# Eden-Kramer-Lab/spectral_connectivity

Measured on AMD Instinct MI355X. Metric: channel-pair*freq-bins/s for CSM+coherence(+wPLI), higher is better.
Workload: dtype f32

## Files before the change

### spectral_connectivity_amd/_build.py

```python
import hashlib
import os
import shutil
import subprocess
import sys
from concurrent.futures import ThreadPoolExecutor

HERE = os.path.dirname(os.path.abspath(__file__))
CSRC = os.path.join(HERE, "csrc")
LIB = os.path.join(HERE, "libsc_hip.so")
OBJ_DIR = os.path.join(os.path.dirname(HERE), "build", "obj")
SOURCES = ["sc_api.hip", "sc_taper.hip", "sc_mtfft.hip", "sc_mtfft_long.hip", "sc_mtfft_mixed.hip", "sc_mtfft_f64.hip", "sc_csm.hip", "sc_nonlinear.hip", "sc_fused.hip", "sc_fused2.hip", "sc_measure.hip",
           "sc_wilson.hip", "sc_wilson_fft.hip", "sc_wilson_pair.hip", "sc_mvar.hip", "sc_conditional.hip", "sc_blockwise.hip", "sc_global.hip", "sc_canonical.hip", "sc_partial.hip", "sc_jackknife.hip", "sc_f64.hip",
           "sc_timing.hip", "sc_memory.hip", "sc_comm.hip"]
HEADERS = ["sc_common.h", "sc_stage.h", "sc_fused_common.h", "sc_fused_plan.h", "sc_jacobi.h", "sc_wilson_fft.h", "sc_wilson_loop.h", "sc_complex.h", "sc_mtfft_bfly.h", os.path.join("..", "..", "include", "sc_hip.h")]
FLAGS = ["-O3", "-std=c++17", "--offload-arch=gfx950", "-fPIC", "-Wno-unused-result", "-fno-slp-vectorize"]


def _hipcc():
    for cand in (os.environ.get("HIPCC"), shutil.which("hipcc"), "/opt/rocm/bin/hipcc"):
        if cand and os.path.exists(cand):
            return cand
    raise RuntimeError("hipcc not found: cannot build libsc_hip.so (set HIPCC=/path/to/hipcc)")


def sources():
    return [os.path.join(CSRC, s) for s in SOURCES if os.path.exists(os.path.join(CSRC, s))]


def is_stale():
# ... 55 lines not shown
```

### spectral_connectivity_amd/csrc/sc_api.hip

```cpp
#include <stdarg.h>
#include <stdlib.h>
#include <string.h>
#include <rocfft/rocfft.h>
#include "sc_common.h"

static thread_local char g_err[512] = "";

void sc_set_error(const char* fmt, ...) {
    va_list ap;
    va_start(ap, fmt);
    vsnprintf(g_err, sizeof(g_err), fmt, ap);
    va_end(ap);
}

static const char* const g_switch_names[SC_SW_COUNT] = {
    "SC_FUSED_DEBUG", "SC_FUSED2_TERMS", "SC_FUSED_SPLIT", "SC_FUSED_NO_SMALL", "SC_MTFFT_DEBUG", "SC_MTFFT_WIDE", "SC_MTFFT_F64",
    "SC_F64_SPLIT", "SC_F64_OC", "SC_F64_NO_FORK", "SC_F64_NO_BLOCK", "SC_WILSON_FFT", "SC_GLOBAL_EIG", "SC_GLOBAL_NT256",
    "SC_GRANGER_KERNEL", "SC_FUSED_FOLD_OBS", "SC_MTFFT_LONG", "SC_CANON_EIG", "SC_MTFFT_MIXED", "SC_MTFFT_MIXED_GEO", "SC_MTFFT_SLICE", "SC_MVAR_INVERSE"};
static char g_switch_val[SC_SW_COUNT][32];
static bool g_switch_set[SC_SW_COUNT];
extern "C" int sc_debug_reload_env(void) {
    for (int i = 0; i < SC_SW_COUNT; ++i) {
        const char* v = getenv(g_switch_names[i]);
        g_switch_set[i] = v != nullptr;
        if (v) { strncpy(g_switch_val[i], v, sizeof(g_switch_val[i]) - 1); g_switch_val[i][sizeof(g_switch_val[i]) - 1] = 0; }
    }
    return SC_OK;
}
static const int g_switches_loaded = sc_debug_reload_env();
const char* sc_switch(int id) { return (id >= 0 && id < SC_SW_COUNT && g_switch_set[id]) ? g_switch_val[id] : nullptr; }

#include <mutex>
#include <vector>
// ... 254 lines not shown
```

### spectral_connectivity_amd/csrc/sc_common.h

```cpp
#pragma once
#include <hip/hip_runtime.h>
#include <stdint.h>
#include <stdio.h>
#include "../../include/sc_hip.h"
#include "sc_complex.h"

void sc_set_error(const char* fmt, ...);
struct ScRec;
struct ScCsmView;

enum ScSwitch {
    SC_SW_FUSED_DEBUG, SC_SW_FUSED2_TERMS, SC_SW_FUSED_SPLIT, SC_SW_FUSED_NO_SMALL, SC_SW_MTFFT_DEBUG, SC_SW_MTFFT_WIDE,
    SC_SW_MTFFT_F64, SC_SW_F64_SPLIT, SC_SW_F64_OC, SC_SW_F64_NO_FORK, SC_SW_F64_NO_BLOCK, SC_SW_WILSON_FFT, SC_SW_GLOBAL_EIG,
    SC_SW_GLOBAL_NT256, SC_SW_GRANGER_KERNEL, SC_SW_FUSED_FOLD_OBS, SC_SW_MTFFT_LONG, SC_SW_CANON_EIG, SC_SW_MTFFT_MIXED, SC_SW_MTFFT_MIXED_GEO, SC_SW_MTFFT_SLICE, SC_SW_MVAR_INVERSE, SC_SW_COUNT
};
const char* sc_switch(int id);

int sc_internal_rows_to_bins(const void* d_Z, void* d_X, int64_t rows, int64_t F, int64_t batch, int64_t b_off,
                             int64_t nyquist_row, hipStream_t st);

bool sc_internal_mtfft_long_applies(int64_t N, int64_t C, int64_t groups);
int64_t sc_internal_mtfft_long_coverage(int64_t N, int64_t C);
int sc_internal_mtfft_long(const float* d_x, int64_t T, int64_t R, int64_t C, int64_t L, int64_t step, int64_t W, int64_t N,
                           const float* d_tapers, int64_t K, int detrend_type, const void* d_twiddles, void* d_X, void* d_P,
                           const float* d_scale, hipStream_t st);

bool sc_internal_mtfft_mix_has(int64_t N);
bool sc_internal_mtfft_mix_applies(int64_t N, int64_t C, int64_t groups);
int64_t sc_internal_mtfft_mix_coverage(int64_t N, int64_t C, bool planes);
// ... 237 lines not shown
```

### spectral_connectivity_amd/csrc/sc_fused.hip

```cpp
#include <stdlib.h>
#include "sc_stage.h"
#include "sc_fused_common.h"

#ifdef FU_TRACE
__device__ unsigned long long fu_trace_buf[12 * 4];
#define FU_T0() unsigned long long fu_t = __builtin_readcyclecounter()
#define FU_TICK(slot)                                                                  \
    do {                                                                               \
        const unsigned long long fu_n = __builtin_readcyclecounter();                  \
        if (blockIdx.x == 0 && (threadIdx.x & 63) == 0) fu_trace_buf[(threadIdx.x >> 6) * 4 + (slot)] += fu_n - fu_t; \
        fu_t = fu_n;                                                                   \
    } while (0)
extern "C" int sc_debug_fused_trace(unsigned long long* out, int reset) {
    if (out) (void)hipMemcpyFromSymbol(out, HIP_SYMBOL(fu_trace_buf), sizeof(unsigned long long) * 48);
    if (reset) { unsigned long long z[48] = {0}; (void)hipMemcpyToSymbol(HIP_SYMBOL(fu_trace_buf), z, sizeof z); }
    return 0;
}
#else
#define FU_T0() do {} while (0)
#define FU_TICK(slot) do {} while (0)
#endif

#define FU_PLANE 36
#define FU_CSTRIDE 220
// ... 379 lines not shown
    constexpr int wps = 8 / NSETS;
    const int set = vw / wps, rsub = vw % wps;
    if constexpr (NSETS == 1) {
        fused_valu_body<NB32, COL_LO, ROW_HI, 0, OP>(p, st, planes, raw, tid, vw, rsub, wps, rec, o_lo);
    } else {
        if (set == 0) fused_valu_body<NB32, COL_LO, ROW_HI, 0, OP>(p, st, planes, raw, tid, vw, rsub, wps, rec, o_lo);
        else fused_valu_body<NB32, COL_LO, ROW_HI, 1, OP>(p, st, planes, raw, tid, vw, rsub, wps, rec, o_lo);
    }
}

template <int NB32, int COL_LO, int ROW_HI, int OP>
__global__ void __launch_bounds__(FU_THREADS) fused_csm_absim_kernel(FusedArgs p) {
    extern __shared__ __align__(16) unsigned char smem[];
    const int tid = threadIdx.x;
    const int wave = __builtin_amdgcn_readfirstlane(tid >> 6);
    const int bin = blockIdx.x / p.n_split, part = blockIdx.x - bin * p.n_split;
    const int g = bin / p.F, f = bin - g * p.F;
    ScStage st = p.st;
    st.base = p.st.base + (int64_t)f * st.ax.sF + sc_group_offset(st.ax, g);
    const int nc = (p.st.n_obs + FU_OC - 1) / FU_OC;
    const int o_lo = (int)((int64_t)part * nc / p.n_split) * FU_OC;
    const int o_hi = (int)((int64_t)(part + 1) * nc / p.n_split) * FU_OC;
    st.n_obs = o_hi < p.st.n_obs ? o_hi : p.st.n_obs;
    float* rec = (part == 0 ? p.accum : p.ws + (int64_t)(part - 1) * p.n_bins * p.floats_per_bin) +
                 (int64_t)bin * p.floats_per_bin;
    unsigned short* planes = reinterpret_cast<unsigned short*>(smem);
    constexpr size_t plane_bytes = (size_t)2 * NB32 * 32 * FU_CSTRIDE * 2;
    constexpr size_t red_bytes = (size_t)4 * FU_MAXB * 16 * 64 * sizeof(float);
    float* raw = reinterpret_cast<float*>(smem + (plane_bytes > red_bytes ? plane_bytes : red_bytes));
    if (wave < 4) {
        if (p.debug_skip & 32) __builtin_amdgcn_s_setprio(2);
        fused_mfma_role<NB32>(p, st, planes, raw, tid, wave, rec, o_lo);
    } else {
        if (p.debug_skip & 16) __builtin_amdgcn_s_setprio(2);
        fused_valu_role<NB32, COL_LO, ROW_HI, OP>(p, st, planes, raw, tid, wave - 4, rec, o_lo);
    }
}

__global__ void __launch_bounds__(256) fused_fold_kernel(FusedArgs p) {
    const int64_t plane = (int64_t)p.n_tiles * SC_TILE_ELEMS;
// ... 35 lines not shown
        SC_CHECK_HIP(hipGetLastError());
        return SC_OK;
    }
};

#define SM_THREADS 448
#define SM_CHUNK_BYTES (24 * 1024)

template <bool ABS, bool SQ, bool SGN>
struct SmallSlots { static constexpr int NQ = 2 + (ABS ? 1 : 0) + (SQ ? 1 : 0) + (SGN ? 1 : 0); };

template <bool ABS, bool SQ, bool SGN, bool NORM>
__global__ void __launch_bounds__(SM_THREADS) small_csm_absim_kernel(FusedArgs p) {
    extern __shared__ __align__(16) unsigned char smem[];
    const int tid = threadIdx.x;
    const int bin = blockIdx.x / p.n_split, part = blockIdx.x - bin * p.n_split;
    const int g = bin / p.F, f = bin - g * p.F;
    ScStage st = p.st;
    st.base = p.st.base + (int64_t)f * st.ax.sF + sc_group_offset(st.ax, g);
    const int nc32 = (p.st.n_obs + FU_OC - 1) / FU_OC;
    const int o_lo = (int)((int64_t)part * nc32 / p.n_split) * FU_OC;
    int o_hi = (int)((int64_t)(part + 1) * nc32 / p.n_split) * FU_OC;
    if (o_hi > p.st.n_obs) o_hi = p.st.n_obs;
    float* rec = (part == 0 ? p.accum : p.ws + (int64_t)(part - 1) * p.n_bins * p.floats_per_bin) +
                 (int64_t)bin * p.floats_per_bin;

    const int C = st.C, B = C >> 1, nbk = B * (B + 1) / 2;
    const int S = SM_THREADS / nbk;
    const int s = tid / nbk, b = tid - s * nbk;
    const bool active = s < S;
    int bi = 0, bj = 0;
    { int rem = b, len = B; while (rem >= len) { rem -= len; ++bi; --len; } bj = bi + rem; }
    const int RS = 2 * C;
    const int half = C >> 1;
    int OC = SM_CHUNK_BYTES / (RS * 4);
    OC -= OC % S;
    if (OC > 16 * S) OC = 16 * S;
    const int per_thread = OC / S;
    float* buf0 = reinterpret_cast<float*>(smem);
    float* buf1 = buf0 + (size_t)OC * RS;
// ... 138 lines not shown

static bool fused_ok(const void* d_X, const ScAxes& ax) {
    if (ax.C < 1 || ax.C > 256 || (ax.C & 1)) return false;
    if ((ax.sW | ax.sR | ax.sK | ax.sF) & 1) return false;
    return d_X == nullptr || (((uintptr_t)d_X) % 16 == 0);
}

static bool small_ok(const ScAxes& ax, bool nonlinear_plane) { return ax.C <= (nonlinear_plane ? 48 : 42); }
static bool small_ok_sq(const ScAxes& ax) { return ax.C <= 58; }
static bool small_ok_sign(const ScAxes& ax) { return ax.C <= 44; }

extern "C" int sc_fused_supported(int64_t n_signals) {
    return (n_signals >= 2 && n_signals <= 256 && (n_signals % 2) == 0) ? 1 : 0;
}

int sc_internal_fused_pick_split(int n_bins, int n_obs) {
    const char* e = sc_switch(SC_SW_FUSED_SPLIT);
    const int nc = (n_obs + FU_OC - 1) / FU_OC;
    static int cu_of_device[64] = {0};
    int dev = 0, n_cu = 256;
    if (hipGetDevice(&dev) == hipSuccess && dev >= 0 && dev < 64) {
        if (cu_of_device[dev] == 0) {
            int v = 0;
            cu_of_device[dev] = (hipDeviceGetAttribute(&v, hipDeviceAttributeMultiprocessorCount, dev) == hipSuccess && v > 0) ? v : 256;
        }
        n_cu = cu_of_device[dev];
    }
    int best = 1;
    double best_cost = 1e30;
    for (int S = 1; S <= 24; ++S) {
        if (S > 1 && nc / S < 16) break;
        const double rounds = (double)(((int64_t)n_bins * S + n_cu - 1) / n_cu);
        const double cost = rounds * ((double)nc / S + 3.0) * (1.0 + 0.02 * (S - 1));
        if (cost < best_cost - 1e-9) { best_cost = cost; best = S; }
    }
    if (e && atoi(e) >= 1 && atoi(e) <= 24 && (atoi(e) == 1 || nc / atoi(e) >= 1)) best = atoi(e);
    return best;
}
int sc_internal_fused_set_parts(FusedArgs* a, int n_obs, void* d_workspace, int64_t workspace_bytes) {
    int S = d_workspace ? sc_internal_fused_pick_split(a->n_bins, n_obs) : 1;
    while (S > 1 && (int64_t)(S - 1) * fu_part_bytes(*a) > workspace_bytes) --S;
    SC_REQUIRE(S == 1 || ((uintptr_t)d_workspace % 16) == 0, "workspace must be 16-byte aligned");
    a->n_split = S;
    a->ws = (float*)d_workspace;
    return SC_OK;
}

void sc_internal_fu_assign_rows(FusedArgs* a) {
    const int NB = a->NB, col_lo = a->map.col_lo;
    const int R = a->map.row_hi < NB ? a->map.row_hi : NB;
    auto c0 = [&](int r) { return r > col_lo ? r : col_lo; };
    unsigned packed[4];
    a->seg_n = 0u;
    for (int w = 0; w < 4; ++w) {
        int sg[6] = {0, 0, 0, 0, 0, 0};
        if (R >= 5) {
            const int rA = w, rB = R - 1 - w;
            if (rA <= rB) { sg[0] = rA; sg[1] = c0(rA); sg[2] = NB - c0(rA); }
// ... 52 lines not shown
    } else if (mode == FU_MODE_SIGN) {
        a->csm_plane = a->abs_plane = a->sq_plane = -1;
    } else {
        a->sign_plane = -1;
        if (a->abs_plane < 0) a->sq_plane = -1;
    }
    fu_headline_fold(a);
    return SC_OK;
}

extern "C" int64_t sc_fused_workspace_bytes(const sc_spectra_desc* desc, uint32_t planes) {
    FusedArgs a;
    ScAxes ax;
    const int mode = (planes & SC_PLANE_CSM) ? FU_MODE_CSM : (planes & SC_PLANE_UNIT) ? FU_MODE_UNIT : FU_MODE_SIGN;
    if (fused_setup(nullptr, desc, planes, mode, &a, &ax) != SC_OK) return 0;
    return (int64_t)(sc_internal_fused_pick_split(a.n_bins, ax.n_obs) - 1) * fu_part_bytes(a);
}

static int fused_run(const void* d_X, const sc_spectra_desc* desc, uint32_t planes, int mode, float* d_accum,
                     void* d_workspace, int64_t workspace_bytes, void* d_scratch, int64_t scratch_bytes, void* stream) {
    ScTimed timed_("fused_stage_b", stream);
    SC_REQUIRE(d_X && desc && d_accum, "NULL argument");
    FusedArgs a;
    ScAxes ax;
    const bool unit = mode == FU_MODE_UNIT;
    const int rc = fused_setup(d_X, desc, planes, mode, &a, &ax);
    if (rc != SC_OK) return rc;
    a.accum = d_accum;
    a.st.base = (const float2*)d_X;
    a.st.ax = ax;
    a.st.obs_stride = sc_stage_linear_stride(ax);
// ... 58 lines not shown
```

### spectral_connectivity_amd/csrc/sc_fused2.hip

```cpp
#include <stdlib.h>
#include "sc_fused_common.h"

typedef _Float16 h16x4 __attribute__((ext_vector_type(4)));
typedef _Float16 h16x8 __attribute__((ext_vector_type(8)));
typedef _Float16 h16x2 __attribute__((ext_vector_type(2)));
typedef __attribute__((address_space(3))) unsigned char lds_u8;
typedef short s16x4 __attribute__((ext_vector_type(4)));
typedef __attribute__((address_space(3))) s16x4 lds_s16x4;

#define F2_GROUP 1056
#define F2_PLANE (8 * F2_GROUP + 64)
#define F2_NPL 6
#define F2_HPL 4
#define F2_BUF (F2_NPL * F2_PLANE)
#define F2_NBUF 3
#define F2_SCALE_OFF (F2_NBUF * F2_BUF)
#define F2_LDS (F2_SCALE_OFF + 512)
#define F2_ROW_TILE 256

extern "C" int64_t sc_planes_scales_work_bytes(int64_t n_rows, int64_t width);
extern "C" int64_t sc_planes_row_bytes(int64_t n_signals) { return (int64_t)F2_ROW_TILE * ((n_signals + 31) / 32); }

__device__ __forceinline__ unsigned f2_pack(float lo, float hi) {
    const h16x2 v = {(_Float16)lo, (_Float16)hi};
// ... 617 lines not shown
        const double cyc = (double)(h[s * 4 + 2] - h[s * 4]), ticks = (double)(h[s * 4 + 3] - h[s * 4 + 1]);
        if (ticks > 0 && cyc > 0) { sum += cyc / (ticks / 100.0e6) * 1e-9; ++n; }
    }
    if (ghz) *ghz = n ? sum / n : 0.0;
    return SC_OK;
}

template <int NB32, int COL_LO, int ROW_HI, int OP>
__global__ void __launch_bounds__(FU_THREADS) fused2_kernel(Fused2Args a) {
    extern __shared__ __align__(16) unsigned char smem[];
    const FusedArgs& p = a.f;
    const int tid = threadIdx.x;
    const int wave = __builtin_amdgcn_readfirstlane(tid >> 6);
    const int clock_slot = blockIdx.x == 0 ? 0 : (blockIdx.x == gridDim.x / 2 ? 1 : (blockIdx.x == gridDim.x - 1 ? 2 : -1));
    if (clock_slot >= 0 && tid == 0) f2_clock_stamp(clock_slot, 0);
    const int bin = blockIdx.x / p.n_split, part = blockIdx.x - bin * p.n_split;
    const int g = bin / p.F, f = bin - g * p.F;
    const int nc = (p.st.n_obs + FU_OC - 1) / FU_OC;
    const int o_lo = (int)((int64_t)part * nc / p.n_split) * FU_OC;
    int o_hi = (int)((int64_t)(part + 1) * nc / p.n_split) * FU_OC;
    if (o_hi > p.st.n_obs) o_hi = p.st.n_obs;
    const int n_part = o_hi - o_lo;
    float* rec = (part == 0 ? p.accum : p.ws + (int64_t)(part - 1) * p.n_bins * p.floats_per_bin) + (int64_t)bin * p.floats_per_bin;
    const unsigned char* part_base = a.P + ((int64_t)f * p.st.ax.sF + sc_group_offset(p.st.ax, g) + (int64_t)o_lo * a.obs_rows) * a.row_bytes;
    lds_u8* lds = (lds_u8*)smem;
    constexpr int NHALF = NB32 <= 2 ? 2 : 1, CH = FU_OC * NHALF;
    const F2Loader L = f2_loader<NHALF>(a, wave, part_base);
    for (int i = tid * 16; i < F2_SCALE_OFF; i += FU_THREADS * 16)
        *reinterpret_cast<u32x4*>(smem + i) = (u32x4){0u, 0u, 0u, 0u};
    if (tid < 128) {
        const int gch = fu_byte(p.map.off32, tid >> 5) * 32 + (tid & 31);
        reinterpret_cast<float*>(smem + F2_SCALE_OFF)[tid] = ((tid >> 5) < p.NB32 && (tid & 31) < fu_byte(p.map.n32, tid >> 5) && gch < p.st.C)
                                                                 ? a.inv_scale[gch] : 1.f;
    }
    __syncthreads();
    f2_issue<NHALF>(a, L, lds, 0, n_part);
    const bool second = n_part > CH && !(p.debug_skip & 8);
    if (second) f2_issue<NHALF>(a, L, lds + F2_BUF, CH, n_part - CH);
// ... 144 lines not shown
```

### spectral_connectivity_amd/csrc/sc_fused_common.h

```cpp
#pragma once
#include "sc_stage.h"
#include "sc_fused_plan.h"

typedef float f32x4 __attribute__((ext_vector_type(4)));
typedef short bf16x8 __attribute__((ext_vector_type(8)));
typedef unsigned int u32x4 __attribute__((ext_vector_type(4)));
typedef float f32x2 __attribute__((ext_vector_type(2)));
typedef float f32x16 __attribute__((ext_vector_type(16)));

#define FU_OC 32
#define FU_THREADS 768
#define FU_MAXB 5
#define FU_FLUSH 16

struct FuMap {
    unsigned off32, n32, t32;
    int NBr;
    int col_lo, row_hi;
};
__host__ __device__ inline int fu_byte(unsigned packed, int b) { return (int)((packed >> (8 * b)) & 0xffu); }
__host__ __device__ inline int fu_gt(const FuMap& m, int b) { return fu_byte(m.t32, b >> 1) + (b & 1); }
__host__ __device__ inline bool fu_tile_ok(const FuMap& m, int b) { return (b & 1) * 16 < fu_byte(m.n32, b >> 1); }

struct FusedArgs {
    ScStage st;
    FuMap map;
    float* accum;
    int64_t floats_per_bin;
    int n_bins, F, NB, n_tiles, NB32, n_blocks32, n_sets;
    int shape_col_lo, shape_row_hi;
    int csm_plane, abs_plane;
    int sq_plane, sign_plane;
    int fold[6], n_fold;
    int nl_op;
    unsigned seg0, seg1, seg2, seg3, seg_n;
    int n_split;
    float* ws;
    int debug_skip;
};

__device__ __forceinline__ unsigned cvt_pk_bf16(float lo, float hi) {
    unsigned r;
    asm("v_cvt_pk_bf16_f32 %0, %1, %2" : "=v"(r) : "v"(lo), "v"(hi));
    return r;
}
__device__ __forceinline__ float bf16lo_to_f32(unsigned p) { return __uint_as_float(p << 16); }
__device__ __forceinline__ float bf16hi_to_f32(unsigned p) { return __uint_as_float(p & 0xffff0000u); }

__device__ __forceinline__ void split4(const float x[4], uint2& h, uint2& m, uint2& l) {
    h.x = cvt_pk_bf16(x[0], x[1]); h.y = cvt_pk_bf16(x[2], x[3]);
    const float r0 = x[0] - bf16lo_to_f32(h.x), r1 = x[1] - bf16hi_to_f32(h.x);
    const float r2 = x[2] - bf16lo_to_f32(h.y), r3 = x[3] - bf16hi_to_f32(h.y);
    m.x = cvt_pk_bf16(r0, r1); m.y = cvt_pk_bf16(r2, r3);
    const float s0 = r0 - bf16lo_to_f32(m.x), s1 = r1 - bf16hi_to_f32(m.x);
    const float s2 = r2 - bf16lo_to_f32(m.y), s3 = r3 - bf16hi_to_f32(m.y);
    l.x = cvt_pk_bf16(s0, s1); l.y = cvt_pk_bf16(s2, s3);
}

__device__ __forceinline__ int fu_lane() {
    int l;
    asm volatile("v_mbcnt_lo_u32_b32 %0, -1, 0\n\tv_mbcnt_hi_u32_b32 %0, -1, %0" : "=v"(l));
    return l;
}
enum { FU_OP_ABS = 0, FU_OP_SQ = 1, FU_OP_SIGN = 2, FU_OP_UNIT = 3 };

#define FU_BARRIER() asm volatile("s_waitcnt lgkmcnt(0)\n\ts_barrier" ::: "memory")
#define F2_BARRIER() FU_BARRIER()
static_assert(2 * 4 + 1 <= FU_FLUSH, "one fold slot per tile of a wave");

__host__ __device__ constexpr int fu_nblocks(int nb32, int col_lo, int row_hi) {
    int n = 0;
    for (int bi = 0; bi < nb32 && bi < row_hi; ++bi)
        for (int bj = bi > col_lo ? bi : col_lo; bj < nb32; ++bj) ++n;
    return n;
}
__host__ __device__ constexpr int fu_nsets(int nb32, int col_lo, int row_hi) {
    return fu_nblocks(nb32, col_lo, row_hi) > 4 ? 2 : 1;
// ... 62 lines not shown
#pragma unroll
        for (int e = 0; e < 16; ++e) acc[e] = fu_accumulate<OP>(acc[e], d[e]);
    } else {
        acc[0] = fu_accumulate<OP>(acc[0], d[0]);
        __builtin_amdgcn_sched_barrier(0);
#pragma unroll
        for (int e = 1; e < 16; ++e) {
            int a = __float_as_int(acc[e]), t;
            asm("v_med3_i32 %1, %2, -1, 1\n\tv_add_u32 %0, %0, %1" : "+v"(a), "=&v"(t) : "v"(d[e]));
            acc[e] = __int_as_float(a);
        }
    }
}


int sc_internal_fused_pick_split(int n_bins, int n_obs);
int sc_internal_fused_set_parts(FusedArgs* a, int n_obs, void* d_workspace, int64_t workspace_bytes);
void sc_internal_fu_assign_rows(FusedArgs* a);
int sc_internal_fused_combine(const FusedArgs& a, hipStream_t stream);

inline int64_t fu_part_bytes(const FusedArgs& a) { return (int64_t)a.n_bins * a.floats_per_bin * (int64_t)sizeof(float); }

inline void fu_record_geometry(FusedArgs* a, const ScAxes& ax, uint32_t planes) {
    auto offset = [&](uint32_t plane) { return (planes & plane) ? sc_plane_offset(planes, plane) : -1; };
    a->NB = sc_n_blocks(ax.C);
    a->n_tiles = sc_n_tiles(a->NB);
    a->NB32 = (ax.C + 31) / 32;
    a->map.NBr = a->NB;
    a->n_bins = ax.n_groups * ax.F;
    a->F = ax.F;
    a->floats_per_bin = (int64_t)sc_plane_count(planes) * a->n_tiles * SC_TILE_ELEMS;
    a->csm_plane = offset(SC_PLANE_CSM);
    a->abs_plane = offset(SC_PLANE_ABS_IM);
    a->sq_plane = offset(SC_PLANE_IM_SQ);
    a->sign_plane = offset(SC_PLANE_SIGN_IM);
    a->nl_op = FU_OP_ABS;
    a->n_split = 1;
    a->ws = nullptr;
}
inline void fu_headline_fold(FusedArgs* a) {
    a->n_fold = 0;
    if (a->csm_plane >= 0) { a->fold[a->n_fold++] = a->csm_plane; a->fold[a->n_fold++] = a->csm_plane + 1; }
    if (a->abs_plane >= 0) a->fold[a->n_fold++] = a->abs_plane;
}
inline FusedArgs fu_plane_pass(const FusedArgs& a, int plane, int op) {
    FusedArgs b = a;
    b.csm_plane = -1;
    b.abs_plane = plane;
    b.nl_op = op;
    b.fold[0] = plane;
    b.n_fold = 1;
    return b;
// ... 53 lines not shown
```

### spectral_connectivity_amd/csrc/sc_measure.hip

```cpp
#include <math.h>
#include "sc_common.h"

#define SC_EPS64 2.220446049250313e-16

template <typename AccT>
struct RecT {
    const AccT* p;
    __device__ RecT operator+(int64_t n) const { return RecT{p + n}; }
    __device__ double operator[](int64_t i) const { return (double)p[i]; }
};

template <typename AccT>
struct RecPartsT {
    const AccT* p;
    const AccT* q;
    int n_parts;
    int64_t stride;
    __device__ RecPartsT operator+(int64_t n) const { return RecPartsT{p + n, q + n, n_parts, stride}; }
    __device__ double operator[](int64_t i) const {
        AccT s = p[i];
        for (int k = 1; k < n_parts; ++k) s += q[i + (k - 1) * stride];
        return (double)s;
    }
};

struct MeasureArgs {
    ScRec accum;
    int n_parts;
    const void* rest;
    int64_t part_stride;
    void* out;
    int64_t n_bins, floats_per_bin, total;
    int C, NB, n_tiles;
    int p_csm, p_abs, p_sq, p_sign, p_unit;
    double n_obs, rn_obs;
    int measure;
    int n_multi;
    int multi[SC_MEASURE_MULTI_MAX];
    void* multi_out[SC_MEASURE_MULTI_MAX];
};

template <typename Rec>
__device__ inline double tile_read(Rec bin_rec, int plane, int n_tiles, int NB, int i, int j,
                                  bool* mirrored) {
    int ti = i >> 4, tj = j >> 4, ii = i & 15, jj = j & 15;
    bool m = (ti > tj) || (ti == tj && ii > jj);
    if (m) { int t = ti; ti = tj; tj = t; t = ii; ii = jj; jj = t; }
    *mirrored = m;
    return bin_rec[((int64_t)plane * n_tiles + sc_tile_index(ti, tj, NB)) * SC_TILE_ELEMS + ii * 16 + jj];
}

template <typename AccT, bool PARTS> struct RecSel { using type = RecT<AccT>; };
template <typename AccT> struct RecSel<AccT, true> { using type = RecPartsT<AccT>; };
template <typename AccT, bool PARTS>
// ... 126 lines not shown
    if (i < a.C && j < a.C) {
        if (COMPLEX_OUT) outc[obase + (int64_t)i * a.C + j] = OutT2{(OutT)direct.x, (OutT)direct.y};
        else outf[obase + (int64_t)i * a.C + j] = (OutT)direct.x;
    }
    if (!dtile) {
        mir[jj * 16 + ii] = measure_value(a.measure, a.n_obs, a.rn_obs, measure_mirror(v), false);
        __syncthreads();
        const int r = tj * 16 + ii, c = ti * 16 + jj;
        if (r < a.C && c < a.C) {
            if (COMPLEX_OUT) outc[obase + (int64_t)r * a.C + c] = OutT2{(OutT)mir[tid].x, (OutT)mir[tid].y};
            else outf[obase + (int64_t)r * a.C + c] = (OutT)mir[tid].x;
        }
    }
}

#ifndef MEASURE_MULTI_TPW
#define MEASURE_MULTI_TPW 1
#endif
template <typename OutT, typename AccT, bool PARTS = false>
__global__ void __launch_bounds__(256) measure_tile_multi_kernel(MeasureArgs a) {
    __shared__ MeasureIn raw[256];
    __shared__ double mir[256];
    const int tid = threadIdx.x, ii = tid >> 4, jj = tid & 15;
    const int64_t bin = blockIdx.x;
    using Rec = typename RecSel<AccT, PARTS>::type;
    const Rec rec = make_rec<AccT, PARTS>(a) + bin * a.floats_per_bin;
    const int64_t plane = (int64_t)a.n_tiles * SC_TILE_ELEMS;
    const int64_t obase = bin * (int64_t)a.C * a.C;
    int ti = 0, len = a.NB, t = blockIdx.y * MEASURE_MULTI_TPW;
    while (t >= len) { t -= len; ++ti; --len; }
    for (int u = 0; u < MEASURE_MULTI_TPW; ++u) {
        const int tile_id = blockIdx.y * MEASURE_MULTI_TPW + u;
        if (tile_id >= a.n_tiles) break;
        const int tj = ti + t;
        const Rec tile = rec + ((int64_t)tile_id * SC_TILE_ELEMS + ii * 16 + jj);
        MeasureIn v = {0, 0, 0, 0, 0, 0, 0, 0, 0};
        if (a.p_csm >= 0) {
            v.s_re = (double)tile[a.p_csm * plane];
            v.s_im = (double)tile[(a.p_csm + 1) * plane];
            v.p_i = (double)rec[a.p_csm * plane + (int64_t)sc_tile_index(ti, ti, a.NB) * SC_TILE_ELEMS + ii * 17];
            v.p_j = (double)rec[a.p_csm * plane + (int64_t)sc_tile_index(tj, tj, a.NB) * SC_TILE_ELEMS + jj * 17];
        }
        if (a.p_abs >= 0) v.sa = (double)tile[a.p_abs * plane];
        if (a.p_sq >= 0) v.sq = (double)tile[a.p_sq * plane];
        if (a.p_sign >= 0) v.sg = (double)tile[a.p_sign * plane];
        if (a.p_unit >= 0) {
            v.u_re = (double)tile[a.p_unit * plane];
            v.u_im = (double)tile[(a.p_unit + 1) * plane];
        }
        const bool dtile = ti == tj;
        if (dtile) {
            raw[tid] = v;
            __syncthreads();
            if (ii > jj) v = measure_mirror(raw[jj * 16 + ii]);
            __syncthreads();
        }
        const int i = ti * 16 + ii, j = tj * 16 + jj;
        for (int m = 0; m < a.n_multi; ++m) {
            OutT* outf = (OutT*)a.multi_out[m];
            const int w = a.multi[m];
#ifdef MEASURE_AB_NOMATH
            const double direct = v.s_re + v.sa + w;
#else
            const double direct = measure_value(w, a.n_obs, a.rn_obs, v, i == j).x;
#endif
            if (i < a.C && j < a.C) outf[obase + (int64_t)i * a.C + j] = (OutT)direct;
            if (!dtile) {
                const double sgn = (w == SC_M_COHERENCE_PHASE || w == SC_M_PLI || w == SC_M_WPLI) ? -1.0 : 1.0;
                mir[jj * 16 + ii] = sgn * direct;
                __syncthreads();
                const int r = tj * 16 + ii, c = ti * 16 + jj;
                if (r < a.C && c < a.C) outf[obase + (int64_t)r * a.C + c] = (OutT)mir[tid];
                __syncthreads();
            }
        }
        if (++t >= len) { t = 0; ++ti; --len; }
    }
}

static uint32_t measure_needs(int measure) {
    switch (measure) {
    case SC_M_POWER: case SC_M_CSM: case SC_M_COHERENCY: case SC_M_COHERENCE_MAGNITUDE:
    case SC_M_COHERENCE_PHASE: case SC_M_IMAGINARY_COHERENCE: return SC_PLANE_CSM;
    case SC_M_PLV: case SC_M_PLV_COMPLEX: case SC_M_PPC: return SC_PLANE_UNIT;
    case SC_M_PLI: case SC_M_DEBIASED_PLI2: return SC_PLANE_SIGN_IM;
    case SC_M_WPLI: return SC_PLANE_CSM | SC_PLANE_ABS_IM;
    case SC_M_DEBIASED_WPLI2: return SC_PLANE_CSM | SC_PLANE_ABS_IM | SC_PLANE_IM_SQ;
    }
    return 0;
}

// ... 34 lines not shown
    a.n_multi = n_measures;
    if ((planes & need) != need) {
        sc_set_error("measures need accumulator planes 0x%x, record has 0x%x", need, planes);
        return SC_EINVAL;
    }
    a.p_csm = (need & SC_PLANE_CSM) ? sc_plane_offset(planes, SC_PLANE_CSM) : -1;
    a.p_abs = (need & SC_PLANE_ABS_IM) ? sc_plane_offset(planes, SC_PLANE_ABS_IM) : -1;
    a.p_sq = (need & SC_PLANE_IM_SQ) ? sc_plane_offset(planes, SC_PLANE_IM_SQ) : -1;
    a.p_sign = (need & SC_PLANE_SIGN_IM) ? sc_plane_offset(planes, SC_PLANE_SIGN_IM) : -1;
    a.p_unit = (need & SC_PLANE_UNIT) ? sc_plane_offset(planes, SC_PLANE_UNIT) : -1;
    a.n_obs = (double)n_observations;
    a.rn_obs = 1.0 / a.n_obs;
    a.measure = measures[0];
    a.total = n_bins * n_signals * n_signals;
    SC_REQUIRE(n_bins < (int64_t)1 << 31 && a.n_tiles <= 65535, "output too large for one launch");
    const dim3 grid((unsigned)n_bins, (unsigned)((a.n_tiles + MEASURE_MULTI_TPW - 1) / MEASURE_MULTI_TPW));
    hipStream_t st = (hipStream_t)stream;
    if (n_parts > 1) {
        if (a.accum.f64) {
            if (wide) hipLaunchKernelGGL((measure_tile_multi_kernel<double, double, true>), grid, dim3(256), 0, st, a);
            else hipLaunchKernelGGL((measure_tile_multi_kernel<float, double, true>), grid, dim3(256), 0, st, a);
        } else {
            if (wide) hipLaunchKernelGGL((measure_tile_multi_kernel<double, float, true>), grid, dim3(256), 0, st, a);
            else hipLaunchKernelGGL((measure_tile_multi_kernel<float, float, true>), grid, dim3(256), 0, st, a);
        }
        SC_CHECK_HIP(hipGetLastError());
        return SC_OK;
    }
    if (a.accum.f64) {
        if (wide) hipLaunchKernelGGL((measure_tile_multi_kernel<double, double>), grid, dim3(256), 0, st, a);
        else hipLaunchKernelGGL((measure_tile_multi_kernel<float, double>), grid, dim3(256), 0, st, a);
// ... 124 lines not shown
```

Before: 2.693 billion.

## Add tapered observation split planner and vectorized 32x32 measure tile kernel

```diff
diff --git a/spectral_connectivity_amd/_build.py b/spectral_connectivity_amd/_build.py
--- a/spectral_connectivity_amd/_build.py
+++ b/spectral_connectivity_amd/_build.py
@@ -12,7 +12,7 @@
 SOURCES = ["sc_api.hip", "sc_taper.hip", "sc_mtfft.hip", "sc_mtfft_long.hip", "sc_mtfft_mixed.hip", "sc_mtfft_f64.hip", "sc_csm.hip", "sc_nonlinear.hip", "sc_fused.hip", "sc_fused2.hip", "sc_measure.hip",
            "sc_wilson.hip", "sc_wilson_fft.hip", "sc_wilson_pair.hip", "sc_mvar.hip", "sc_conditional.hip", "sc_blockwise.hip", "sc_global.hip", "sc_canonical.hip", "sc_partial.hip", "sc_jackknife.hip", "sc_f64.hip",
            "sc_timing.hip", "sc_memory.hip", "sc_comm.hip"]
-HEADERS = ["sc_common.h", "sc_stage.h", "sc_fused_common.h", "sc_fused_plan.h", "sc_jacobi.h", "sc_wilson_fft.h", "sc_wilson_loop.h", "sc_complex.h", "sc_mtfft_bfly.h", os.path.join("..", "..", "include", "sc_hip.h")]
+HEADERS = ["sc_common.h", "sc_stage.h", "sc_fused_common.h", "sc_fused_plan.h", "sc_fused_split.h", "sc_jacobi.h", "sc_wilson_fft.h", "sc_wilson_loop.h", "sc_complex.h", "sc_mtfft_bfly.h", os.path.join("..", "..", "include", "sc_hip.h")]
 FLAGS = ["-O3", "-std=c++17", "--offload-arch=gfx950", "-fPIC", "-Wno-unused-result", "-fno-slp-vectorize"]
 
 
diff --git a/spectral_connectivity_amd/csrc/sc_api.hip b/spectral_connectivity_amd/csrc/sc_api.hip
--- a/spectral_connectivity_amd/csrc/sc_api.hip
+++ b/spectral_connectivity_amd/csrc/sc_api.hip
@@ -16,7 +16,7 @@
 static const char* const g_switch_names[SC_SW_COUNT] = {
     "SC_FUSED_DEBUG", "SC_FUSED2_TERMS", "SC_FUSED_SPLIT", "SC_FUSED_NO_SMALL", "SC_MTFFT_DEBUG", "SC_MTFFT_WIDE", "SC_MTFFT_F64",
     "SC_F64_SPLIT", "SC_F64_OC", "SC_F64_NO_FORK", "SC_F64_NO_BLOCK", "SC_WILSON_FFT", "SC_GLOBAL_EIG", "SC_GLOBAL_NT256",
-    "SC_GRANGER_KERNEL", "SC_FUSED_FOLD_OBS", "SC_MTFFT_LONG", "SC_CANON_EIG", "SC_MTFFT_MIXED", "SC_MTFFT_MIXED_GEO", "SC_MTFFT_SLICE", "SC_MVAR_INVERSE"};
+    "SC_GRANGER_KERNEL", "SC_FUSED_FOLD_OBS", "SC_MTFFT_LONG", "SC_CANON_EIG", "SC_MTFFT_MIXED", "SC_MTFFT_MIXED_GEO", "SC_MTFFT_SLICE", "SC_MVAR_INVERSE", "SC_FUSED_SPLIT_TAIL"};
 static char g_switch_val[SC_SW_COUNT][32];
 static bool g_switch_set[SC_SW_COUNT];
 extern "C" int sc_debug_reload_env(void) {
diff --git a/spectral_connectivity_amd/csrc/sc_common.h b/spectral_connectivity_amd/csrc/sc_common.h
--- a/spectral_connectivity_amd/csrc/sc_common.h
+++ b/spectral_connectivity_amd/csrc/sc_common.h
@@ -12,7 +12,7 @@
 enum ScSwitch {
     SC_SW_FUSED_DEBUG, SC_SW_FUSED2_TERMS, SC_SW_FUSED_SPLIT, SC_SW_FUSED_NO_SMALL, SC_SW_MTFFT_DEBUG, SC_SW_MTFFT_WIDE,
     SC_SW_MTFFT_F64, SC_SW_F64_SPLIT, SC_SW_F64_OC, SC_SW_F64_NO_FORK, SC_SW_F64_NO_BLOCK, SC_SW_WILSON_FFT, SC_SW_GLOBAL_EIG,
-    SC_SW_GLOBAL_NT256, SC_SW_GRANGER_KERNEL, SC_SW_FUSED_FOLD_OBS, SC_SW_MTFFT_LONG, SC_SW_CANON_EIG, SC_SW_MTFFT_MIXED, SC_SW_MTFFT_MIXED_GEO, SC_SW_MTFFT_SLICE, SC_SW_MVAR_INVERSE, SC_SW_COUNT
+    SC_SW_GLOBAL_NT256, SC_SW_GRANGER_KERNEL, SC_SW_FUSED_FOLD_OBS, SC_SW_MTFFT_LONG, SC_SW_CANON_EIG, SC_SW_MTFFT_MIXED, SC_SW_MTFFT_MIXED_GEO, SC_SW_MTFFT_SLICE, SC_SW_MVAR_INVERSE, SC_SW_FUSED_SPLIT_TAIL, SC_SW_COUNT
 };
 const char* sc_switch(int id);
 
diff --git a/spectral_connectivity_amd/csrc/sc_fused.hip b/spectral_connectivity_amd/csrc/sc_fused.hip
--- a/spectral_connectivity_amd/csrc/sc_fused.hip
+++ b/spectral_connectivity_amd/csrc/sc_fused.hip
@@ -417,16 +417,13 @@
     extern __shared__ __align__(16) unsigned char smem[];
     const int tid = threadIdx.x;
     const int wave = __builtin_amdgcn_readfirstlane(tid >> 6);
-    const int bin = blockIdx.x / p.n_split, part = blockIdx.x - bin * p.n_split;
+    const FuPart pr = fu_part_range(p, blockIdx.x);
+    const int bin = pr.bin, o_lo = pr.o_lo;
     const int g = bin / p.F, f = bin - g * p.F;
     ScStage st = p.st;
     st.base = p.st.base + (int64_t)f * st.ax.sF + sc_group_offset(st.ax, g);
-    const int nc = (p.st.n_obs + FU_OC - 1) / FU_OC;
-    const int o_lo = (int)((int64_t)part * nc / p.n_split) * FU_OC;
-    const int o_hi = (int)((int64_t)(part + 1) * nc / p.n_split) * FU_OC;
-    st.n_obs = o_hi < p.st.n_obs ? o_hi : p.st.n_obs;
-    float* rec = (part == 0 ? p.accum : p.ws + (int64_t)(part - 1) * p.n_bins * p.floats_per_bin) +
-                 (int64_t)bin * p.floats_per_bin;
+    st.n_obs = pr.o_hi;
+    float* rec = fu_part_record(p, pr);
     unsigned short* planes = reinterpret_cast<unsigned short*>(smem);
     constexpr size_t plane_bytes = (size_t)2 * NB32 * 32 * FU_CSTRIDE * 2;
     constexpr size_t red_bytes = (size_t)4 * FU_MAXB * 16 * 64 * sizeof(float);
@@ -492,16 +489,12 @@
 __global__ void __launch_bounds__(SM_THREADS) small_csm_absim_kernel(FusedArgs p) {
     extern __shared__ __align__(16) unsigned char smem[];
     const int tid = threadIdx.x;
-    const int bin = blockIdx.x / p.n_split, part = blockIdx.x - bin * p.n_split;
+    const FuPart pr = fu_part_range(p, blockIdx.x);
+    const int bin = pr.bin, o_lo = pr.o_lo, o_hi = pr.o_hi;
     const int g = bin / p.F, f = bin - g * p.F;
     ScStage st = p.st;
     st.base = p.st.base + (int64_t)f * st.ax.sF + sc_group_offset(st.ax, g);
-    const int nc32 = (p.st.n_obs + FU_OC - 1) / FU_OC;
-    const int o_lo = (int)((int64_t)part * nc32 / p.n_split) * FU_OC;
-    int o_hi = (int)((int64_t)(part + 1) * nc32 / p.n_split) * FU_OC;
-    if (o_hi > p.st.n_obs) o_hi = p.st.n_obs;
-    float* rec = (part == 0 ? p.accum : p.ws + (int64_t)(part - 1) * p.n_bins * p.floats_per_bin) +
-                 (int64_t)bin * p.floats_per_bin;
+    float* rec = fu_part_record(p, pr);
 
     const int C = st.C, B = C >> 1, nbk = B * (B + 1) / 2;
     const int S = SM_THREADS / nbk;
@@ -670,9 +663,14 @@
     return (n_signals >= 2 && n_signals <= 256 && (n_signals % 2) == 0) ? 1 : 0;
 }
 
-int sc_internal_fused_pick_split(int n_bins, int n_obs) {
+void sc_internal_fused_pick_split(int n_bins, int n_obs, FuSplitPlan* plan) {
     const char* e = sc_switch(SC_SW_FUSED_SPLIT);
     const int nc = (n_obs + FU_OC - 1) / FU_OC;
+    if (e) {
+        const char* t = sc_switch(SC_SW_FUSED_SPLIT_TAIL);
+        const int tail = t ? atoi(t) : 0;
+        if (fu_split_forced(nc, atoi(e), tail > 0 ? tail : 0, plan)) return;
+    }
     static int cu_of_device[64] = {0};
     int dev = 0, n_cu = 256;
     if (hipGetDevice(&dev) == hipSuccess && dev >= 0 && dev < 64) {
@@ -682,22 +680,21 @@
         }
         n_cu = cu_of_device[dev];
     }
-    int best = 1;
-    double best_cost = 1e30;
-    for (int S = 1; S <= 24; ++S) {
-        if (S > 1 && nc / S < 16) break;
-        const double rounds = (double)(((int64_t)n_bins * S + n_cu - 1) / n_cu);
-        const double cost = rounds * ((double)nc / S + 3.0) * (1.0 + 0.02 * (S - 1));
-        if (cost < best_cost - 1e-9) { best_cost = cost; best = S; }
-    }
-    if (e && atoi(e) >= 1 && atoi(e) <= 24 && (atoi(e) == 1 || nc / atoi(e) >= 1)) best = atoi(e);
-    return best;
+    static thread_local struct { int n_bins, nc, n_cu; FuSplitPlan plan; } last = {0, 0, 0, {}};
+    if (last.n_bins != n_bins || last.nc != nc || last.n_cu != n_cu) {
+        fu_split_plan(n_bins, nc, n_cu, &last.plan);
+        last.n_bins = n_bins; last.nc = nc; last.n_cu = n_cu;
+    }
+    *plan = last.plan;
 }
 int sc_internal_fused_set_parts(FusedArgs* a, int n_obs, void* d_workspace, int64_t workspace_bytes) {
-    int S = d_workspace ? sc_internal_fused_pick_split(a->n_bins, n_obs) : 1;
+    FuSplitPlan plan = fu_one_part(n_obs);
+    if (d_workspace) sc_internal_fused_pick_split(a->n_bins, n_obs, &plan);
+    int S = plan.n_parts;
     while (S > 1 && (int64_t)(S - 1) * fu_part_bytes(*a) > workspace_bytes) --S;
+    if (S != plan.n_parts) fu_split_fill(&plan, (n_obs + FU_OC - 1) / FU_OC, S, 0);
     SC_REQUIRE(S == 1 || ((uintptr_t)d_workspace % 16) == 0, "workspace must be 16-byte aligned");
-    a->n_split = S;
+    fu_set_plan(a, plan);
     a->ws = (float*)d_workspace;
     return SC_OK;
 }
@@ -780,7 +777,9 @@
     ScAxes ax;
     const int mode = (planes & SC_PLANE_CSM) ? FU_MODE_CSM : (planes & SC_PLANE_UNIT) ? FU_MODE_UNIT : FU_MODE_SIGN;
     if (fused_setup(nullptr, desc, planes, mode, &a, &ax) != SC_OK) return 0;
-    return (int64_t)(sc_internal_fused_pick_split(a.n_bins, ax.n_obs) - 1) * fu_part_bytes(a);
+    FuSplitPlan plan;
+    sc_internal_fused_pick_split(a.n_bins, ax.n_obs, &plan);
+    return (int64_t)(plan.n_parts - 1) * fu_part_bytes(a);
 }
 
 static int fused_run(const void* d_X, const sc_spectra_desc* desc, uint32_t planes, int mode, float* d_accum,
diff --git a/spectral_connectivity_amd/csrc/sc_fused2.hip b/spectral_connectivity_amd/csrc/sc_fused2.hip
--- a/spectral_connectivity_amd/csrc/sc_fused2.hip
+++ b/spectral_connectivity_amd/csrc/sc_fused2.hip
@@ -655,14 +655,11 @@
     const int wave = __builtin_amdgcn_readfirstlane(tid >> 6);
     const int clock_slot = blockIdx.x == 0 ? 0 : (blockIdx.x == gridDim.x / 2 ? 1 : (blockIdx.x == gridDim.x - 1 ? 2 : -1));
     if (clock_slot >= 0 && tid == 0) f2_clock_stamp(clock_slot, 0);
-    const int bin = blockIdx.x / p.n_split, part = blockIdx.x - bin * p.n_split;
+    const FuPart pr = fu_part_range(p, blockIdx.x);
+    const int bin = pr.bin, o_lo = pr.o_lo;
     const int g = bin / p.F, f = bin - g * p.F;
-    const int nc = (p.st.n_obs + FU_OC - 1) / FU_OC;
-    const int o_lo = (int)((int64_t)part * nc / p.n_split) * FU_OC;
-    int o_hi = (int)((int64_t)(part + 1) * nc / p.n_split) * FU_OC;
-    if (o_hi > p.st.n_obs) o_hi = p.st.n_obs;
-    const int n_part = o_hi - o_lo;
-    float* rec = (part == 0 ? p.accum : p.ws + (int64_t)(part - 1) * p.n_bins * p.floats_per_bin) + (int64_t)bin * p.floats_per_bin;
+    const int n_part = pr.o_hi - o_lo;
+    float* rec = fu_part_record(p, pr);
     const unsigned char* part_base = a.P + ((int64_t)f * p.st.ax.sF + sc_group_offset(p.st.ax, g) + (int64_t)o_lo * a.obs_rows) * a.row_bytes;
     lds_u8* lds = (lds_u8*)smem;
     constexpr int NHALF = NB32 <= 2 ? 2 : 1, CH = FU_OC * NHALF;
diff --git a/spectral_connectivity_amd/csrc/sc_fused_common.h b/spectral_connectivity_amd/csrc/sc_fused_common.h
--- a/spectral_connectivity_amd/csrc/sc_fused_common.h
+++ b/spectral_connectivity_amd/csrc/sc_fused_common.h
@@ -1,6 +1,7 @@
 #pragma once
 #include "sc_stage.h"
 #include "sc_fused_plan.h"
+#include "sc_fused_split.h"
 
 typedef float f32x4 __attribute__((ext_vector_type(4)));
 typedef short bf16x8 __attribute__((ext_vector_type(8)));
@@ -35,6 +36,8 @@
     int nl_op;
     unsigned seg0, seg1, seg2, seg3, seg_n;
     int n_split;
+    int n_big;
+    int n_chunks, tail;
     float* ws;
     int debug_skip;
 };
@@ -61,6 +64,20 @@
     int l;
     asm volatile("v_mbcnt_lo_u32_b32 %0, -1, 0\n\tv_mbcnt_hi_u32_b32 %0, -1, %0" : "=v"(l));
     return l;
+}
+struct FuPart { int bin, part, o_lo, o_hi; };
+__device__ __forceinline__ FuPart fu_part_range(const FusedArgs& p, int block) {
+    FuPart r;
+    const int n_front = p.n_bins * p.n_big;
+    r.bin = block < n_front ? block / p.n_big : block - n_front;
+    r.part = block < n_front ? block - r.bin * p.n_big : p.n_split - 1;
+    r.o_lo = fu_split_bound(r.part, p.n_big, p.n_chunks, p.tail) * FU_OC;
+    r.o_hi = fu_split_bound(r.part + 1, p.n_big, p.n_chunks, p.tail) * FU_OC;
+    if (r.o_hi > p.st.n_obs) r.o_hi = p.st.n_obs;
+    return r;
+}
+__device__ __forceinline__ float* fu_part_record(const FusedArgs& p, const FuPart& r) {
+    return (r.part == 0 ? p.accum : p.ws + (int64_t)(r.part - 1) * p.n_bins * p.floats_per_bin) + (int64_t)r.bin * p.floats_per_bin;
 }
 enum { FU_OP_ABS = 0, FU_OP_SQ = 1, FU_OP_SIGN = 2, FU_OP_UNIT = 3 };
 
@@ -153,13 +170,24 @@
 }
 
 
-int sc_internal_fused_pick_split(int n_bins, int n_obs);
+void sc_internal_fused_pick_split(int n_bins, int n_obs, FuSplitPlan* plan);
 int sc_internal_fused_set_parts(FusedArgs* a, int n_obs, void* d_workspace, int64_t workspace_bytes);
 void sc_internal_fu_assign_rows(FusedArgs* a);
 int sc_internal_fused_combine(const FusedArgs& a, hipStream_t stream);
 
 inline int64_t fu_part_bytes(const FusedArgs& a) { return (int64_t)a.n_bins * a.floats_per_bin * (int64_t)sizeof(float); }
 
+inline void fu_set_plan(FusedArgs* a, const FuSplitPlan& plan) {
+    a->n_split = plan.n_parts;
+    a->n_big = plan.tail ? plan.n_parts - 1 : plan.n_parts;
+    a->n_chunks = plan.bound[plan.n_parts];
+    a->tail = plan.tail;
+}
+inline FuSplitPlan fu_one_part(int n_obs) {
+    FuSplitPlan plan;
+    fu_split_fill(&plan, (n_obs + FU_OC - 1) / FU_OC, 1, 0);
+    return plan;
+}
 inline void fu_record_geometry(FusedArgs* a, const ScAxes& ax, uint32_t planes) {
     auto offset = [&](uint32_t plane) { return (planes & plane) ? sc_plane_offset(planes, plane) : -1; };
     a->NB = sc_n_blocks(ax.C);
@@ -174,7 +202,7 @@
     a->sq_plane = offset(SC_PLANE_IM_SQ);
     a->sign_plane = offset(SC_PLANE_SIGN_IM);
     a->nl_op = FU_OP_ABS;
-    a->n_split = 1;
+    fu_set_plan(a, fu_one_part(ax.n_obs));
     a->ws = nullptr;
 }
 inline void fu_headline_fold(FusedArgs* a) {
diff --git a/spectral_connectivity_amd/csrc/sc_fused_split.h b/spectral_connectivity_amd/csrc/sc_fused_split.h
--- /dev/null
+++ b/spectral_connectivity_amd/csrc/sc_fused_split.h
@@ -0,0 +1,112 @@
+#pragma once
+#include <stdint.h>
+
+enum {
+    FU_SPLIT_MAX = 24,
+    FU_SPLIT_MIN_BIG = 16,
+    FU_SPLIT_FIXED = 3,
+    FU_SPLIT_CANDIDATES = 256,
+    FU_SPLIT_TAPER_ROUNDS = 7
+};
+
+struct FuSplitPlan {
+    int n_parts, tail;
+    int bound[FU_SPLIT_MAX + 1];
+    double makespan;
+};
+
+inline double fu_split_part_factor(int n_parts) { return 1.0 + 0.02 * (n_parts - 1); }
+
+#ifdef __HIPCC__
+__host__ __device__
+#endif
+inline int fu_split_bound(int k, int n_big, int n_chunks, int tail) {
+    return k < n_big ? (int)((int64_t)k * (n_chunks - tail) / n_big) : (k == n_big ? n_chunks - tail : n_chunks);
+}
+inline void fu_split_fill(FuSplitPlan* p, int n_chunks, int n_parts, int tail) {
+    p->n_parts = n_parts;
+    p->tail = n_parts > 1 ? tail : 0;
+    const int n_big = p->tail ? n_parts - 1 : n_parts, big_chunks = n_chunks - p->tail;
+    for (int k = 0; k <= FU_SPLIT_MAX; ++k) p->bound[k] = n_chunks;
+    for (int k = 0; k < n_big; ++k) p->bound[k] = (int)((int64_t)k * big_chunks / n_big);
+    if (p->tail) p->bound[n_big] = big_chunks;
+    p->makespan = 0.0;
+}
+
+inline double fu_split_equal_cost(int n_bins, int n_chunks, int n_cu, int S) {
+    const double rounds = (double)(((int64_t)n_bins * S + n_cu - 1) / n_cu);
+    return rounds * ((double)n_chunks / S + FU_SPLIT_FIXED) * fu_split_part_factor(S);
+}
+inline int fu_split_equal_parts(int n_bins, int n_chunks, int n_cu) {
+    int best = 1;
+    double best_cost = 1e30;
+    for (int S = 1; S <= FU_SPLIT_MAX; ++S) {
+        if (S > 1 && n_chunks / S < FU_SPLIT_MIN_BIG) break;
+        const double cost = fu_split_equal_cost(n_bins, n_chunks, n_cu, S);
+        if (cost < best_cost - 1e-9) { best_cost = cost; best = S; }
+    }
+    return best;
+}
+inline double fu_split_equal_floor(int n_bins, int n_chunks, int n_cu, int S) {
+    const int64_t rounds = ((int64_t)n_bins * S + n_cu - 1) / n_cu;
+    const double by_rounds = (double)(rounds * (n_chunks / S + FU_SPLIT_FIXED));
+    const double by_work = (double)((int64_t)n_bins * (n_chunks + (int64_t)FU_SPLIT_FIXED * S)) / n_cu;
+    return (by_rounds > by_work ? by_rounds : by_work) * fu_split_part_factor(S);
+}
+
+inline double fu_split_tapered_cost(int n_bins, int n_cu, int S, int big, int tail) {
+    const int64_t cb = big + FU_SPLIT_FIXED, ct = tail + FU_SPLIT_FIXED;
+    const int64_t B = (int64_t)n_bins * (S - 1), R = B / n_cu, r = B % n_cu, P = n_cu, nb = n_bins;
+    int64_t U;
+    if (r == 0) {
+        U = R * cb + (nb + P - 1) / P * ct;
+    } else {
+        const int64_t low = P - r, q = (cb + ct - 1) / ct, hole = low * q, high = (R + 1) * cb;
+        if (nb <= hole) {
+            const int64_t filled = R * cb + (nb + low - 1) / low * ct;
+            U = filled > high ? filled : high;
+        } else {
+            const int64_t d = R * cb + q * ct - high, left = nb - hole, m = left / P, rem = left % P;
+            U = rem == 0 ? high + d + m * ct : rem <= r ? high + (m + 1) * ct : high + d + (m + 1) * ct;
+        }
+    }
+    return (double)U * fu_split_part_factor(S);
+}
+
+inline void fu_split_plan(int n_bins, int n_chunks, int n_cu, FuSplitPlan* out) {
+    if (n_bins < 1) n_bins = 1;
+    if (n_chunks < 1) n_chunks = 1;
+    if (n_cu < 1) n_cu = 1;
+    const int S_eq = fu_split_equal_parts(n_bins, n_chunks, n_cu);
+    const double floor_eq = fu_split_equal_floor(n_bins, n_chunks, n_cu, S_eq);
+    const bool taper = ((int64_t)n_bins * S_eq + n_cu - 1) / n_cu <= FU_SPLIT_TAPER_ROUNDS;
+    int best_S = 0, best_big = 0;
+    double best = 0.99 * floor_eq;
+    for (int S = 2; taper && S <= FU_SPLIT_MAX; ++S) {
+        int lo = n_chunks / S + 1;
+        if (lo < FU_SPLIT_MIN_BIG) lo = FU_SPLIT_MIN_BIG;
+        const int hi = (n_chunks - 1) / (S - 1);
+        if (hi < lo) continue;
+        const int step = (hi - lo + FU_SPLIT_CANDIDATES) / FU_SPLIT_CANDIDATES;
+        for (int big = lo; big <= hi; big += step) {
+            const double cost = fu_split_tapered_cost(n_bins, n_cu, S, big, n_chunks - big * (S - 1));
+            if (cost < best - 1e-9) { best = cost; best_S = S; best_big = big; }
+        }
+    }
+    if (best_S) {
+        fu_split_fill(out, n_chunks, best_S, n_chunks - best_big * (best_S - 1));
+        out->makespan = best;
+    } else {
+        fu_split_fill(out, n_chunks, S_eq, 0);
+        out->makespan = fu_split_equal_cost(n_bins, n_chunks, n_cu, S_eq);
+    }
+}
+
+inline bool fu_split_forced(int n_chunks, int n_parts, int tail, FuSplitPlan* out) {
+    if (n_parts < 1 || n_parts > FU_SPLIT_MAX || tail < 0) return false;
+    if (n_parts == 1) { fu_split_fill(out, n_chunks, 1, 0); return true; }
+    const int n_big = tail ? n_parts - 1 : n_parts;
+    if ((n_chunks - tail) / n_big < 1) return false;
+    fu_split_fill(out, n_chunks, n_parts, tail);
+    return true;
+}
diff --git a/spectral_connectivity_amd/csrc/sc_measure.hip b/spectral_connectivity_amd/csrc/sc_measure.hip
--- a/spectral_connectivity_amd/csrc/sc_measure.hip
+++ b/spectral_connectivity_amd/csrc/sc_measure.hip
@@ -38,6 +38,7 @@
     int n_multi;
     int multi[SC_MEASURE_MULTI_MAX];
     void* multi_out[SC_MEASURE_MULTI_MAX];
+    int vec_out;
 };
 
 template <typename Rec>
@@ -194,67 +195,97 @@
     }
 }
 
-#ifndef MEASURE_MULTI_TPW
-#define MEASURE_MULTI_TPW 1
-#endif
 template <typename OutT, typename AccT, bool PARTS = false>
 __global__ void __launch_bounds__(256) measure_tile_multi_kernel(MeasureArgs a) {
-    __shared__ MeasureIn raw[256];
-    __shared__ double mir[256];
-    const int tid = threadIdx.x, ii = tid >> 4, jj = tid & 15;
+    typedef AccT AccV __attribute__((ext_vector_type(4)));
+    typedef OutT OutV __attribute__((ext_vector_type(4)));
+    __shared__ OutT val[SC_MEASURE_MULTI_MAX][32][33];
+    __shared__ double pw[64];
+    const int tid = threadIdx.x, q = tid >> 6, lane = tid & 63, ii = lane >> 2, j4 = (lane & 3) * 4;
     const int64_t bin = blockIdx.x;
-    using Rec = typename RecSel<AccT, PARTS>::type;
-    const Rec rec = make_rec<AccT, PARTS>(a) + bin * a.floats_per_bin;
+    int bi = 0, len = (a.NB + 1) / 2, t = blockIdx.y;
+    while (t >= len) { t -= len; ++bi; --len; }
+    const int bj = bi + t;
+    const int ti = 2 * bi + (q >> 1), tj = 2 * bj + (q & 1);
+    const bool have = ti <= tj && tj < a.NB;
     const int64_t plane = (int64_t)a.n_tiles * SC_TILE_ELEMS;
+    const int64_t toff = have ? (int64_t)sc_tile_index(ti, tj, a.NB) * SC_TILE_ELEMS + ii * 16 + j4 : 0;
+    const int pch = (lane < 32 ? 32 * bi : 32 * bj - 32) + lane, ptile = pch >> 4;
+    const bool pw_ok = q == 0 && a.p_csm >= 0 && ptile < a.NB;
+    const int64_t poff = pw_ok ? a.p_csm * plane + (int64_t)sc_tile_index(ptile, ptile, a.NB) * SC_TILE_ELEMS + (pch & 15) * 17 : 0;
+    const int n_parts = PARTS ? a.n_parts : 1;
+    const AccV zero = {0, 0, 0, 0};
+    AccV s_re = zero, s_im = zero, s_sa = zero, s_sq = zero, s_sg = zero, s_ur = zero, s_ui = zero;
+    AccT s_pw = 0;
+    for (int k = 0; k < n_parts; ++k) {
+        const AccT* r = (k == 0 ? (const AccT*)a.accum.p : (const AccT*)a.rest + (int64_t)(k - 1) * a.part_stride) + bin * a.floats_per_bin;
+        AccV l_re = zero, l_im = zero, l_sa = zero, l_sq = zero, l_sg = zero, l_ur = zero, l_ui = zero;
+        AccT l_pw = 0;
+        if (have) {
+            if (a.p_csm >= 0) {
+                l_re = *reinterpret_cast<const AccV*>(r + a.p_csm * plane + toff);
+                l_im = *reinterpret_cast<const AccV*>(r + (a.p_csm + 1) * plane + toff);
+            }
+            if (a.p_abs >= 0) l_sa = *reinterpret_cast<const AccV*>(r + a.p_abs * plane + toff);
+            if (a.p_sq >= 0) l_sq = *reinterpret_cast<const AccV*>(r + a.p_sq * plane + toff);
+            if (a.p_sign >= 0) l_sg = *reinterpret_cast<const AccV*>(r + a.p_sign * plane + toff);
+            if (a.p_unit >= 0) {
+                l_ur = *reinterpret_cast<const AccV*>(r + a.p_unit * plane + toff);
+                l_ui = *reinterpret_cast<const AccV*>(r + (a.p_unit + 1) * plane + toff);
+            }
+        }
+        if (pw_ok) l_pw = r[poff];
+        if (k == 0) { s_re = l_re; s_im = l_im; s_sa = l_sa; s_sq = l_sq; s_sg = l_sg; s_ur = l_ur; s_ui = l_ui; s_pw = l_pw; }
+        else { s_re += l_re; s_im += l_im; s_sa += l_sa; s_sq += l_sq; s_sg += l_sg; s_ur += l_ur; s_ui += l_ui; s_pw += l_pw; }
+    }
+    if (q == 0) pw[lane] = (double)s_pw;
+    __syncthreads();
+    const int r_blk = (q >> 1) * 16 + ii, i = 32 * bi + r_blk;
+    if (have) {
+#pragma unroll
+        for (int e = 0; e < 4; ++e) {
+            const int c_blk = (q & 1) * 16 + j4 + e, j = 32 * bj + c_blk;
+            if (i > j) continue;
+            MeasureIn v = {(double)s_re[e], (double)s_im[e], pw[r_blk], pw[32 + c_blk], (double)s_sa[e], (double)s_sq[e], (double)s_sg[e],
+                           (double)s_ur[e], (double)s_ui[e]};
+            for (int m = 0; m < a.n_multi; ++m) {
+#ifdef MEASURE_AB_NOMATH
+                val[m][r_blk][c_blk] = (OutT)(v.s_re + v.sa + a.multi[m]);
+#else
+                val[m][r_blk][c_blk] = (OutT)measure_value(a.multi[m], a.n_obs, a.rn_obs, v, i == j).x;
+#endif
+            }
+        }
+    }
+    __syncthreads();
+    const int r = tid >> 3, c0 = (tid & 7) * 4;
     const int64_t obase = bin * (int64_t)a.C * a.C;
-    int ti = 0, len = a.NB, t = blockIdx.y * MEASURE_MULTI_TPW;
-    while (t >= len) { t -= len; ++ti; --len; }
-    for (int u = 0; u < MEASURE_MULTI_TPW; ++u) {
-        const int tile_id = blockIdx.y * MEASURE_MULTI_TPW + u;
-        if (tile_id >= a.n_tiles) break;
-        const int tj = ti + t;
-        const Rec tile = rec + ((int64_t)tile_id * SC_TILE_ELEMS + ii * 16 + jj);
-        MeasureIn v = {0, 0, 0, 0, 0, 0, 0, 0, 0};
-        if (a.p_csm >= 0) {
-            v.s_re = (double)tile[a.p_csm * plane];
-            v.s_im = (double)tile[(a.p_csm + 1) * plane];
-            v.p_i = (double)rec[a.p_csm * plane + (int64_t)sc_tile_index(ti, ti, a.NB) * SC_TILE_ELEMS + ii * 17];
-            v.p_j = (double)rec[a.p_csm * plane + (int64_t)sc_tile_index(tj, tj, a.NB) * SC_TILE_ELEMS + jj * 17];
-        }
-        if (a.p_abs >= 0) v.sa = (double)tile[a.p_abs * plane];
-        if (a.p_sq >= 0) v.sq = (double)tile[a.p_sq * plane];
-        if (a.p_sign >= 0) v.sg = (double)tile[a.p_sign * plane];
-        if (a.p_unit >= 0) {
-            v.u_re = (double)tile[a.p_unit * plane];
-            v.u_im = (double)tile[(a.p_unit + 1) * plane];
-        }
-        const bool dtile = ti == tj;
-        if (dtile) {
-            raw[tid] = v;
-            __syncthreads();
-            if (ii > jj) v = measure_mirror(raw[jj * 16 + ii]);
-            __syncthreads();
-        }
-        const int i = ti * 16 + ii, j = tj * 16 + jj;
-        for (int m = 0; m < a.n_multi; ++m) {
-            OutT* outf = (OutT*)a.multi_out[m];
-            const int w = a.multi[m];
-#ifdef MEASURE_AB_NOMATH
-            const double direct = v.s_re + v.sa + w;
-#else
-            const double direct = measure_value(w, a.n_obs, a.rn_obs, v, i == j).x;
-#endif
-            if (i < a.C && j < a.C) outf[obase + (int64_t)i * a.C + j] = (OutT)direct;
-            if (!dtile) {
-                const double sgn = (w == SC_M_COHERENCE_PHASE || w == SC_M_PLI || w == SC_M_WPLI) ? -1.0 : 1.0;
-                mir[jj * 16 + ii] = sgn * direct;
-                __syncthreads();
-                const int r = tj * 16 + ii, c = ti * 16 + jj;
-                if (r < a.C && c < a.C) outf[obase + (int64_t)r * a.C + c] = (OutT)mir[tid];
-                __syncthreads();
-            }
-        }
-        if (++t >= len) { t = 0; ++ti; --len; }
+    auto put = [&](OutT* out, int row, int col, const OutT x[4]) {
+        if (row >= a.C) return;
+        OutT* dst = out + obase + (int64_t)row * a.C + col;
+        if (a.vec_out) {
+            if (col >= a.C) return;
+            const OutV xv = {x[0], x[1], x[2], x[3]};
+            *reinterpret_cast<OutV*>(dst) = xv;
+        } else {
+#pragma unroll
+            for (int e = 0; e < 4; ++e)
+                if (col + e < a.C) dst[e] = x[e];
+        }
+    };
+    for (int m = 0; m < a.n_multi; ++m) {
+        const int w = a.multi[m];
+        const OutT sgn = (w == SC_M_COHERENCE_PHASE || w == SC_M_PLI || w == SC_M_WPLI) ? (OutT)-1 : (OutT)1;
+        OutT* out = (OutT*)a.multi_out[m];
+        OutT x[4];
+#pragma unroll
+        for (int e = 0; e < 4; ++e) x[e] = (bi < bj || r <= c0 + e) ? val[m][r][c0 + e] : sgn * val[m][c0 + e][r];
+        put(out, 32 * bi + r, 32 * bj + c0, x);
+        if (bi < bj) {
+#pragma unroll
+            for (int e = 0; e < 4; ++e) x[e] = sgn * val[m][c0 + e][r];
+            put(out, 32 * bj + r, 32 * bi + c0, x);
+        }
     }
 }
 
@@ -319,7 +350,15 @@
     a.measure = measures[0];
     a.total = n_bins * n_signals * n_signals;
     SC_REQUIRE(n_bins < (int64_t)1 << 31 && a.n_tiles <= 65535, "output too large for one launch");
-    const dim3 grid((unsigned)n_bins, (unsigned)((a.n_tiles + MEASURE_MULTI_TPW - 1) / MEASURE_MULTI_TPW));
+    const uintptr_t rec_align = 4 * (a.accum.f64 ? sizeof(double) : sizeof(float));
+    SC_REQUIRE((uintptr_t)d_accum % rec_align == 0 && (n_parts == 1 || ((uintptr_t)d_rest % rec_align == 0 && part_stride % 4 == 0)),
+               "records must be aligned to four of their elements");
+    const uintptr_t out_align = 4 * (wide ? sizeof(double) : sizeof(float));
+    a.vec_out = n_signals % 4 == 0 ? 1 : 0;
+    for (int m = 0; m < n_measures; ++m)
+        if ((uintptr_t)d_outs[m] % out_align) a.vec_out = 0;
+    const int nb32 = (a.NB + 1) / 2;
+    const dim3 grid((unsigned)n_bins, (unsigned)(nb32 * (nb32 + 1) / 2));
     hipStream_t st = (hipStream_t)stream;
     if (n_parts > 1) {
         if (a.accum.f64) {
```

After: 2.744 billion, median of 6. No clear change (+1.9%).
